# egordm/tch-geometric

Measured on AMD Instinct MI355X. Metric: sampled edges/sec, neighbor_sampling_homogenous fanout [15,10] on RMAT-24, higher is better.
Workload: dtype int64

## Files before the change

### tch-geometric_amd/csrc/ns_homo_win.hip

```cpp
#include <stdlib.h>

#include <algorithm>
#include <mutex>
#include <type_traits>

#include "ns_tickets.h"
#include "stage_bits.h"
#include "tg_device.h"
#include "tg_host.h"

namespace tg {

constexpr int WIN_PART_BLOCKS = 512;
constexpr int WIN_PART_THREADS = 512;
constexpr int WIN_TILE = 4096;
constexpr int WIN_MAX_BUCKETS = 8192;
constexpr int WIN_MAX_ROWS = 1024;
constexpr int WIN_MAX_PARTS = 16;

struct WinState {
    int64_t begin, end, ne, fbase;
};

struct WinQueues {
// ... 665 lines not shown
    return v ? atoi(v) : dflt;
}

struct WinTuning {
    int64_t window_bytes;
    int32_t gather_blocks, gather_threads, emit_threads, direct_hop0, fuse_first_hops, fold_hist, emit_blocks;
    int32_t staged, stage_round_chunks, stage_gather_threads, stage_gather_blocks, stage_emit_threads, stage_parts, stage_part_min_batches, stage_sort_blocks;
    int32_t stage_fine, stage_concurrent, stage_split, stage_split_round_chunks, store_align64, stage_fine_sub_bits, stage_fine_blocks;
};
static WinTuning &win_tuning() {
    static WinTuning t = {
        (int64_t)win_env_int("TG_WIN_KIB", 512) * 1024,
        win_env_int("TG_WIN_GATHER_BLOCKS", 256),
        win_env_int("TG_WIN_GATHER_THREADS", 512),
        win_env_int("TG_WIN_EMIT_THREADS", 256),
        win_env_int("TG_WIN_DIRECT_HOP0", 1),
        win_env_int("TG_WIN_FUSE_FIRST_HOPS", 1),
        win_env_int("TG_WIN_FOLD_HIST", 1),
        win_env_int("TG_WIN_EMIT_BLOCKS", 768),
        win_env_int("TG_WIN_STAGED", 2),
        win_env_int("TG_WIN_STAGE_ROUND_CHUNKS", 2),
        win_env_int("TG_WIN_STAGE_GATHER_THREADS", 512),
        win_env_int("TG_WIN_STAGE_GATHER_BLOCKS", 512),
        win_env_int("TG_WIN_STAGE_EMIT_THREADS", 256),
        win_env_int("TG_WIN_STAGE_PARTS", 1),
        win_env_int("TG_WIN_STAGE_PART_MIN_BATCHES", 1024),
        win_env_int("TG_WIN_STAGE_SORT_BLOCKS", 0),
        win_env_int("TG_WIN_STAGE_FINE", 1),
        win_env_int("TG_WIN_STAGE_CONCURRENT", 0),
        win_env_int("TG_WIN_STAGE_SPLIT", 0),
        win_env_int("TG_WIN_STAGE_SPLIT_ROUND_CHUNKS", 4),
        win_env_int("TG_WIN_STORE_ALIGN64", 1),
        win_env_int("TG_WIN_STAGE_FINE_SUB_BITS", 7),
        win_env_int("TG_WIN_STAGE_FINE_BLOCKS", 2048),
    };
    return t;
}

constexpr int WIN_MAX_STAGES = 8 * TG_MAX_HOPS + 2;
struct WinStageClock {
    bool enabled = false;
    int n = 0;
    hipEvent_t ev[WIN_MAX_STAGES + 1] = {};
    char name[WIN_MAX_STAGES][24] = {};
    void begin(hipStream_t s) {
        n = 0;
        if (!enabled) return;
        if (!ev[0])
            for (auto &e : ev) (void)hipEventCreate(&e);
        (void)hipEventRecord(ev[0], s);
    }
    void mark(const char *what, int hop, hipStream_t s) {
        if (!enabled || n >= WIN_MAX_STAGES) return;
        snprintf(name[n], sizeof(name[n]), "%s.h%d", what, hop);
        ++n;
        (void)hipEventRecord(ev[n], s);
    }
};
static WinStageClock &win_clock() {
    static WinStageClock c;
    return c;
}

struct WinLayout {
    size_t state, call_keys, n_items, queues, hist, base, items_in, items_sorted, vtab, fine_tot, fine_start, fine_tile_off, item_keys, stage, total, total_push;
    int64_t max_items;
    int stage_words;
};

static StageBits win_stage_bits(const tg_graph *csc) {
    StageBits sb;
    if (!csc) {
        sb.bv = sb.bp = 32;
        return sb;
    }
    sb.bv = stage_bits_of((uint64_t)std::max<int64_t>(csc->n_major, 1) - 1);
    const int64_t longest = csc->max_degree > 0 ? csc->max_degree : csc->n_edges;
    sb.bp = stage_bits_of((uint64_t)std::max<int64_t>(longest, 1) - 1);
    return sb;
}
static int win_stage_words(const tg_graph *csc, const int64_t *fanout, int32_t n_hops) {
    int64_t k = 0;
    for (int h = 1; h < n_hops; ++h) k = std::max(k, fanout[h]);
    if (n_hops < 2 || k > 32) return 0;
    if (!csc) return 32;
    const int bits = stage_slot_bits((int)k, win_stage_bits(csc));
    return (bits <= 512 && k <= 16) ? 16 : (bits <= 1024 ? 32 : 0);
}

static WinLayout win_layout(const tg_graph *csc, int64_t n_batches, int64_t n_seeds, const int64_t *fanout, int32_t n_hops) {
    WinLayout L;
    int64_t layer = n_seeds, widest = n_seeds;
    for (int h = 0; h + 1 < n_hops; ++h) {
        layer *= fanout[h];
        if (layer > widest) widest = layer;
    }
    L.max_items = n_batches * widest;
    size_t at = 0;
    auto take = [&](size_t bytes) {
        const size_t here = at;
        at += (bytes + 255) & ~(size_t)255;
        return here;
    };
    L.state = take((size_t)n_batches * sizeof(WinState));
    L.call_keys = take((size_t)n_batches * sizeof(CallKey));
    L.n_items = take(TG_MAX_HOPS * sizeof(unsigned long long));
    L.queues = take(WIN_MAX_PARTS * sizeof(WinQueues));
    L.hist = take((size_t)std::max(WIN_MAX_ROWS, WIN_MAX_PARTS * WIN_PART_BLOCKS) * WIN_MAX_BUCKETS * sizeof(uint32_t));
    L.base = take((size_t)WIN_MAX_PARTS * (WIN_MAX_BUCKETS + 8) * sizeof(uint32_t));
    L.items_in = take((size_t)L.max_items * sizeof(WinItemW));
    L.items_sorted = take((size_t)L.max_items * sizeof(WinItemW));
    L.vtab = take((size_t)(WIN_MAX_BUCKETS + 8) * sizeof(uint32_t));
    L.total_push = at;
    L.fine_tot = take((size_t)WIN_MAX_PARTS * (WIN_MAX_BUCKETS / 8 + 8) * WIN_FINE_PER_COARSE_MAX * sizeof(uint32_t));
    L.fine_start = take((size_t)WIN_MAX_PARTS * (WIN_MAX_BUCKETS / 8 + 8) * WIN_FINE_PER_COARSE_MAX * sizeof(uint32_t));
    L.fine_tile_off = take(((size_t)L.max_items / WIN_FINE_TILE + WIN_MAX_PARTS + 1) * WIN_FINE_BINS_MAX * sizeof(uint32_t));
    L.item_keys = take((size_t)L.max_items * sizeof(uint16_t));
    L.stage_words = win_stage_words(csc, fanout, n_hops);
    L.stage = take((size_t)L.max_items * L.stage_words * sizeof(uint32_t));
    L.total = at;
    return L;
}

template <typename Item, int KMAX, bool REPLACE>
static int win_run(WinParams p, int64_t n_batches, const int64_t *fanout, int32_t n_hops, hipStream_t stream) {
    const WinTuning t = win_tuning();
    WinStageClock &clk = win_clock();
    const int gather_blocks = (t.gather_blocks + 7) & ~7;
    const bool fold = t.fold_hist && t.direct_hop0 && t.fuse_first_hops && n_hops > 1;
    const size_t hist_lds = fold ? (size_t)p.n_buckets * sizeof(uint32_t) : 0;
    auto emit_threads_for = [&]() {
        int threads = t.emit_threads;
        while (threads > 64 && win_emit_lds_bytes(p.kmax, threads / 64) + hist_lds > 64 * 1024)
            threads = ((threads >> 1) + 63) & ~63;
        return threads;
    };
    p.n_batches = n_batches;
    p.n_rows = (int32_t)std::min<int64_t>(std::min(std::max(t.emit_blocks, 1), WIN_MAX_ROWS), n_batches);
    auto pitch_of = [&](int h) {
        int64_t f = p.n_seeds;
        for (int j = 0; j < h; ++j) f *= fanout[j];
        return f;
    };
    clk.begin(stream);
    int h0 = 0;
    if (t.direct_hop0 && t.fuse_first_hops) {
        const int threads = emit_threads_for();
        if (fold) {
            p.item_pitch = pitch_of(1);
            hipLaunchKernelGGL((win_first_hops_fold_kernel<Item, KMAX, REPLACE>), dim3((unsigned)p.n_rows), dim3(threads),
                               win_emit_lds_bytes(p.kmax, threads / 64) + hist_lds, stream, p, (int)fanout[0], (int)fanout[1]);
        } else {
            TG_HIP(hipMemsetAsync(p.n_items, 0, TG_MAX_HOPS * sizeof(unsigned long long), stream));
            hipLaunchKernelGGL((win_first_hops_kernel<Item, KMAX, REPLACE>), dim3((unsigned)n_batches), dim3(threads),
                               win_emit_lds_bytes(p.kmax, threads / 64), stream, p, (int)fanout[0],
                               n_hops > 1 ? (int)fanout[1] : 0);
        }
        TG_LAUNCH_CHECK();
        clk.mark("first_hops", 0, stream);
        h0 = 1;
    } else {
        hipLaunchKernelGGL(win_init_kernel, dim3((unsigned)n_batches), dim3(256), 0, stream, p, n_batches);
        TG_LAUNCH_CHECK();
        clk.mark("init", 0, stream);
    }
    for (int h = h0; h < n_hops; ++h) {
        p.hop = h;
        p.k = (int32_t)fanout[h];
        p.item_pitch = pitch_of(h);
        const bool emitted = (h == 1 && h0 == 1);
        if (!emitted) {
            const int threads = emit_threads_for();
            if (h == 0 && t.direct_hop0) {
                hipLaunchKernelGGL((win_emit_kernel<Item, KMAX, REPLACE, true>), dim3((unsigned)n_batches), dim3(threads),
                                   win_emit_lds_bytes(p.kmax, threads / 64), stream, p);
                TG_LAUNCH_CHECK();
                clk.mark("emit_direct", h, stream);
                continue;
            }
            if (fold)
                hipLaunchKernelGGL((win_emit_fold_kernel<Item, KMAX, REPLACE>), dim3((unsigned)p.n_rows), dim3(threads),
                                   win_emit_lds_bytes(p.kmax, threads / 64) + hist_lds, stream, p);
            else
                hipLaunchKernelGGL((win_emit_kernel<Item, KMAX, REPLACE, false>), dim3((unsigned)n_batches),
                                   dim3(threads), win_emit_lds_bytes(p.kmax, threads / 64), stream, p);
            TG_LAUNCH_CHECK();
            clk.mark("emit", h, stream);
        }
        if (!fold) {
            hipLaunchKernelGGL(win_hist_kernel<Item>, dim3(WIN_PART_BLOCKS), dim3(WIN_PART_THREADS), 0, stream, p);
            TG_LAUNCH_CHECK();
            clk.mark("hist", h, stream);
        }
        hipLaunchKernelGGL(win_colscan_kernel, dim3((p.n_buckets + 63) / 64), dim3(64 * WIN_SCAN_GROUPS), 0, stream, p,
                           fold ? p.n_rows : WIN_PART_BLOCKS);
        TG_LAUNCH_CHECK();
        hipLaunchKernelGGL(win_basescan_kernel, dim3(1), dim3(1024), 0, stream, p);
        TG_LAUNCH_CHECK();
        clk.mark("scans", h, stream);
        if (fold)
            hipLaunchKernelGGL(win_scatter_fold_kernel<Item>, dim3((unsigned)p.n_rows), dim3(WIN_PART_THREADS), 0, stream, p);
        else
            hipLaunchKernelGGL(win_scatter_kernel<Item>, dim3(WIN_PART_BLOCKS), dim3(WIN_PART_THREADS), 0, stream, p);
        TG_LAUNCH_CHECK();
        clk.mark("scatter", h, stream);
        int gthreads = t.gather_threads;
        while (gthreads > 64 && (size_t)(gthreads / 64) * win_gather_wave_lds_bytes(p.kmax) > 64 * 1024)
            gthreads = ((gthreads >> 1) + 63) & ~63;
        hipLaunchKernelGGL((win_gather_kernel<Item, KMAX, REPLACE>), dim3(gather_blocks), dim3(gthreads),
                           (size_t)(gthreads / 64) * win_gather_wave_lds_bytes(p.kmax), stream, p);
        TG_LAUNCH_CHECK();
        clk.mark("gather", h, stream);
    }
    return TG_OK;
}

constexpr int64_t WIN_STAGED_AUTO_MIN_BATCHES = 2048;
static bool win_staged_wanted(const WinTuning &t, int64_t n_batches, int stage_words) {
    if (t.staged == 2) return n_batches >= WIN_STAGED_AUTO_MIN_BATCHES && stage_words == 16;
    return t.staged != 0;
}
static bool win_staged_applicable(const WinParams &p, const WinTuning &t, const tg_graph *csc, int64_t n_batches,
                                  const int64_t *fanout, int32_t n_hops, int stage_words) {
    if (!win_staged_wanted(t, n_batches, stage_words) || !t.direct_hop0 || n_hops < 2 || stage_words == 0) return false;
    if (csc->n_major >= ((int64_t)1 << 32) || csc->n_edges >= ((int64_t)1 << 32)) return false;
    int64_t pitch = p.n_seeds;
    for (int h = 1; h < n_hops; ++h) {
        pitch *= fanout[h - 1];
        int bits = 1;
        while (((int64_t)1 << bits) < pitch) ++bits;
        if (bits >= 32 || n_batches > ((int64_t)1 << (32 - bits))) return false;
    }
    return true;
}

struct WinSide {
    hipStream_t stream = nullptr;
    hipEvent_t gathered[WIN_MAX_PARTS] = {}, done = nullptr;
    std::mutex mu;
    int ensure() {
        if (stream) return TG_OK;
        int least = 0, greatest = 0;
        const int prio = win_env_int("TG_WIN_SIDE_PRIO", 1);
        if (prio && hipDeviceGetStreamPriorityRange(&least, &greatest) == hipSuccess && greatest < least)
            TG_HIP(hipStreamCreateWithPriority(&stream, hipStreamNonBlocking, prio == 2 ? least : greatest));
        else
            TG_HIP(hipStreamCreateWithFlags(&stream, hipStreamNonBlocking));
        for (auto &e : gathered) TG_HIP(hipEventCreateWithFlags(&e, hipEventDisableTiming));
        TG_HIP(hipEventCreateWithFlags(&done, hipEventDisableTiming));
        return TG_OK;
    }
};
static WinSide &win_side() {
    static WinSide s;
    return s;
}

struct WinDeviceLds {
    int cus, per_cu, per_block;
};
static int win_device_lds(WinDeviceLds *out) {
    constexpr int MAX_DEV = 64;
    static std::mutex mu;
    static WinDeviceLds known[MAX_DEV];
    static bool have[MAX_DEV] = {};
    int dev = 0;
    TG_HIP(hipGetDevice(&dev));
    std::lock_guard<std::mutex> lock(mu);
    if (dev < 0 || dev >= MAX_DEV || !have[dev]) {
        WinDeviceLds d;
        TG_HIP(hipDeviceGetAttribute(&d.cus, hipDeviceAttributeMultiprocessorCount, dev));
        TG_HIP(hipDeviceGetAttribute(&d.per_cu, hipDeviceAttributeMaxSharedMemoryPerMultiprocessor, dev));
        TG_HIP(hipDeviceGetAttribute(&d.per_block, hipDeviceAttributeMaxSharedMemoryPerBlock, dev));
        if (dev < 0 || dev >= MAX_DEV) {
            *out = d;
            return TG_OK;
        }
        known[dev] = d;
        have[dev] = true;
    }
    *out = known[dev];
    return TG_OK;
}

static size_t win_stage_first_lds(int kmax, int threads, int n_coarse, int n_windows, bool narrow) {
    return win_emit_lds_bytes(kmax, threads / 64, WIN_STAGE_FIRST_RC, narrow) + win_stage_tables_bytes(n_coarse, n_windows);
}
static int win_stage_first_threads(int emit_threads, int kmax, int n_coarse, int n_windows, bool narrow) {
    int threads = std::min(emit_threads, WIN_EMIT_MAX_THREADS);
    while (threads > 64 && win_stage_first_lds(kmax, threads, n_coarse, n_windows, narrow) > 64 * 1024)
        threads = ((threads >> 1) + 63) & ~63;
    return threads;
}

struct WinFirstLaunch {
    int32_t rows = 0, per_cu = 0, threads = 0, narrow = 0;
    int64_t lds_bytes = 0;
};
static WinFirstLaunch &win_first_launch() {
    static WinFirstLaunch f;
    return f;
}

template <int W, int KFIRST, int KMAX, bool REPLACE>
static int win_run_staged(WinParams p, const tg_graph *csc, int64_t n_batches, const int64_t *fanout, int32_t n_hops,
                          hipStream_t stream) {
    const WinTuning t = win_tuning();
    WinStageClock &clk = win_clock();
    const StageBits sb = win_stage_bits(csc);
    p.n_windows = (int32_t)((csc->n_edges >> p.shift) + 1);
    auto pitch_of = [&](int h) {
        int64_t f = p.n_seeds;
        for (int j = 0; j < h; ++j) f *= fanout[j];
        return f;
    };
    auto bits_of = [&](int64_t pitch) {
        int bits = 1;
        while (((int64_t)1 << bits) < pitch) ++bits;
        return bits;
    };
    p.n_wbuckets = (p.n_buckets + 63) & ~63;
    p.n_buckets = p.n_wbuckets >> 3;
    const size_t tables = win_stage_tables_bytes(p.n_buckets, p.n_windows);
    int parts = std::min(std::max(t.stage_parts, 1), WIN_MAX_PARTS);
    while (parts > 1 && n_batches / parts < std::max(t.stage_part_min_batches, 1)) --parts;
    if (clk.enabled) parts = 1;
    const bool split = t.stage_split && !clk.enabled;
    if (split) parts = 1;
    WinSide &side = win_side();
    std::unique_lock<std::mutex> side_lock(side.mu, std::defer_lock);
    if (parts > 1 || split) {
        side_lock.lock();
        const int rc = side.ensure();
        if (rc != TG_OK) return rc;
    }
    uint32_t *const hist0 = p.hist, *const base0 = p.base;
    WinQueues *const queues0 = p.queues;
    void *const sorted0 = p.items_sorted, *const in0 = p.items_in;
    uint32_t *const fine_tot0 = p.fine_tot, *const fine_start0 = p.fine_start, *const fine_tile_off0 = p.fine_tile_off;
    const bool first_in_parts = parts > 1 && n_hops == 2;

    WinDeviceLds dl;
    {
        const int rc = win_device_lds(&dl);
        if (rc != TG_OK) return rc;
    }
    const bool narrow_cols = p.ptrs32 != nullptr;
    const int fthreads = win_stage_first_threads(t.emit_threads, p.kmax, p.n_buckets, p.n_windows, narrow_cols);
    const size_t flds = win_stage_first_lds(p.kmax, fthreads, p.n_buckets, p.n_windows, narrow_cols);
    int first_per_cu = 0;
    if (t.stage_sort_blocks <= 0) {
        struct Seen {
            int dev = -1, threads = 0, narrow = 0, per_cu = 0;
            size_t lds = 0;
        };
        static Seen seen;
        static std::mutex seen_mu;
        int dev = 0;
        TG_HIP(hipGetDevice(&dev));
        std::lock_guard<std::mutex> lock(seen_mu);
        if (seen.dev != dev || seen.threads != fthreads || seen.narrow != (int)narrow_cols || seen.lds != flds) {
            const int by_lds = (int)((size_t)dl.per_cu / flds), by_regs = (4 * (512 / 128)) / (fthreads / 64);
            int by_runtime = 0;
            if (narrow_cols)
                TG_HIP(hipOccupancyMaxActiveBlocksPerMultiprocessor(&by_runtime, win_stage_first_kernel<KFIRST, REPLACE, true>, fthreads, flds));
            else
                TG_HIP(hipOccupancyMaxActiveBlocksPerMultiprocessor(&by_runtime, win_stage_first_kernel<KFIRST, REPLACE, false>, fthreads, flds));
            seen.dev = dev;
            seen.threads = fthreads;
            seen.narrow = (int)narrow_cols;
            seen.lds = flds;
            seen.per_cu = std::max(1, std::min(std::min(by_lds, by_regs), by_runtime > 0 ? by_runtime : 1));
        }
        first_per_cu = seen.per_cu;
    }
    const int64_t rows_wanted = t.stage_sort_blocks > 0 ? (int64_t)t.stage_sort_blocks : (int64_t)first_per_cu * std::max(dl.cus, 1);
    auto rows_of = [&](int64_t nb) {
        return (int32_t)std::min<int64_t>(std::min<int64_t>(std::max<int64_t>(rows_wanted, 1), WIN_MAX_ROWS), nb);
    };
    auto part_tables = [&](int part) {
        p.hist = hist0 + (size_t)part * WIN_MAX_ROWS * (WIN_MAX_BUCKETS / 8);
        p.base = base0 + (size_t)part * (WIN_MAX_BUCKETS + 8);
        p.queues = queues0 + part;
    };
    auto launch_first = [&](int part, int64_t b0, int64_t nb, hipStream_t ps) {
        part_tables(part);
        p.b0 = b0;
        p.n_batches = nb;
        p.n_rows = rows_of(nb);
        p.next_pitch = pitch_of(1);
        p.next_idx_bits = bits_of(p.next_pitch);
        if (narrow_cols)
            hipLaunchKernelGGL((win_stage_first_kernel<KFIRST, REPLACE, true>), dim3((unsigned)p.n_rows), dim3(fthreads), flds, ps,
                               p, (int)fanout[0]);
        else
            hipLaunchKernelGGL((win_stage_first_kernel<KFIRST, REPLACE, false>), dim3((unsigned)p.n_rows), dim3(fthreads), flds, ps,
                               p, (int)fanout[0]);
        WinFirstLaunch &fl = win_first_launch();
        fl.rows = p.n_rows;
        fl.per_cu = first_per_cu;
        fl.threads = fthreads;
        fl.narrow = (int32_t)narrow_cols;
        fl.lds_bytes = (int64_t)flds;
    };
    const bool concurrent = first_in_parts && t.stage_concurrent;

    clk.begin(stream);
    hipLaunchKernelGGL(win_vtab_kernel, dim3((p.n_windows + 256) / 256), dim3(256), 0, stream, p, csc->n_major);
    TG_LAUNCH_CHECK();
    if (!first_in_parts) {
        launch_first(0, 0, n_batches, stream);
        TG_LAUNCH_CHECK();
        clk.mark("first", 0, stream);
    }
    if (concurrent) {
        TG_HIP(hipEventRecord(side.gathered[0], stream));
        TG_HIP(hipStreamWaitEvent(side.stream, side.gathered[0], 0));
    }
    for (int h = 1; h < n_hops; ++h) {
        const bool next = h + 1 < n_hops;
        const int hparts = next ? 1 : parts;
        for (int part = 0; part < hparts; ++part) {
            const int64_t b0 = n_batches * part / hparts, nb = n_batches * (part + 1) / hparts - b0;
            const bool counted = h == 1 && (first_in_parts || hparts == 1);
            hipStream_t ps = (concurrent && (part & 1)) ? side.stream : stream;
            if (first_in_parts) {
                launch_first(part, b0, nb, ps);
                TG_LAUNCH_CHECK();
            }
            p.hop = h;
            p.k = (int32_t)fanout[h];
            p.item_pitch = pitch_of(h);
            p.idx_bits = bits_of(p.item_pitch);
            p.next_pitch = next ? pitch_of(h + 1) : 0;
            p.next_idx_bits = next ? bits_of(p.next_pitch) : 0;
            int ethreads = t.stage_emit_threads;
            int rc = std::min(std::max(split ? t.stage_split_round_chunks : t.stage_round_chunks, 1), WIN_STAGE_ROUND_CHUNKS_MAX);
            while (win_stage_emit_lds_bytes(W, p.k, ethreads / 64, rc, split) > 64 * 1024) {
                if (rc > 1)
                    rc >>= 1;
                else if (ethreads > 64)
                    ethreads = ((ethreads >> 1) + 63) & ~63;
                else
                    return tg::fail(TG_ERR_INVALID, "tg_ns_homo_batched_ws: the staged emit kernel does not fit the LDS");
            }
            const size_t elds = win_stage_emit_lds_bytes(W, p.k, ethreads / 64, rc, split);
            int gthreads = t.stage_gather_threads;
            const size_t per_wave = (size_t)(64 * (W + 1) + 64) * sizeof(uint32_t);
            const size_t gcap = std::max<size_t>(64 * 1024, std::min<size_t>((size_t)std::max(dl.per_block, 0), 128 * 1024));
            while (gthreads > 64 && (size_t)(gthreads / 64) * per_wave > gcap) gthreads = ((gthreads >> 1) + 63) & ~63;
            if ((size_t)(gthreads / 64) * per_wave > 64 * 1024) {
                static int raised_on = -1;
                int dev = 0;
                TG_HIP(hipGetDevice(&dev));
                if (raised_on != dev) {
                    TG_HIP(hipFuncSetAttribute(reinterpret_cast<const void *>(&win_stage_gather_kernel<W, KMAX, REPLACE>),
                                               hipFuncAttributeMaxDynamicSharedMemorySize, (int)gcap));
                    raised_on = dev;
                }
            }
            const int gblocks = (std::max(t.stage_gather_blocks, 8) + 7) & ~7;
            part_tables(part);
            p.b0 = b0;
            p.n_batches = nb;
            p.n_rows = rows_of(nb);
            p.items_in = in0;
            p.items_sorted = static_cast<WinItem8 *>(sorted0) + p.b0 * p.item_pitch;
            p.items_fine = static_cast<WinItem8 *>(in0) + p.b0 * p.item_pitch;
            if (!counted) {
                hipLaunchKernelGGL(win_hist8_kernel, dim3((unsigned)p.n_rows), dim3(WIN_PART_THREADS), tables, ps, p);
                TG_LAUNCH_CHECK();
                clk.mark("hist", h, stream);
            }
            hipLaunchKernelGGL(win_colscan_kernel, dim3((p.n_buckets + 63) / 64), dim3(64 * WIN_SCAN_GROUPS), 0, ps, p,
                               p.n_rows);
            TG_LAUNCH_CHECK();
            hipLaunchKernelGGL(win_basescan_kernel, dim3(1), dim3(1024), 0, ps, p);
            TG_LAUNCH_CHECK();
            clk.mark("scans", h, stream);
            {
                static const int tiled = win_env_int("TG_WIN_SCATTER_TILED", 1);
                static const int carry = win_env_int("TG_WIN_SCATTER_CARRY", 1);
                const size_t clds = win_scatter8_carry_lds(WIN_SC_CARRY_TILE, p.n_buckets);
                const size_t ccap = std::max<size_t>(64 * 1024, std::min<size_t>((size_t)std::max(dl.per_block, 0), 128 * 1024));
                if (tiled && carry && p.n_buckets <= WIN_PART_THREADS && clds <= ccap) {
                    if (clds > 64 * 1024) {
                        static int raised_on = -1;
                        int dev = 0;
                        TG_HIP(hipGetDevice(&dev));
                        if (raised_on != dev) {
                            TG_HIP(hipFuncSetAttribute(reinterpret_cast<const void *>(&win_scatter8_carry_kernel<WIN_SC_CARRY_TILE>),
                                                       hipFuncAttributeMaxDynamicSharedMemorySize, (int)ccap));
                            raised_on = dev;
                        }
                    }
                    hipLaunchKernelGGL(win_scatter8_carry_kernel<WIN_SC_CARRY_TILE>, dim3((unsigned)p.n_rows), dim3(WIN_PART_THREADS), clds,
                                       ps, p);
                } else if (tiled && p.n_buckets <= WIN_PART_THREADS && win_scatter8_tiled_lds(p.n_buckets, p.n_windows) <= 64 * 1024)
                    hipLaunchKernelGGL(win_scatter8_tiled_kernel, dim3((unsigned)p.n_rows), dim3(WIN_PART_THREADS),
                                       win_scatter8_tiled_lds(p.n_buckets, p.n_windows), ps, p);
                else
                    hipLaunchKernelGGL(win_scatter8_kernel, dim3((unsigned)p.n_rows), dim3(WIN_PART_THREADS), tables, ps, p);
            }
            TG_LAUNCH_CHECK();
            clk.mark("scatter", h, stream);
            if (t.stage_fine) {
                const int64_t worst = p.n_batches * p.item_pitch;
                const size_t vt = (size_t)(p.n_windows + 1 + p.n_buckets + 1) * sizeof(uint32_t);
                p.fine_sub_bits = std::min(std::max(t.stage_fine_sub_bits, 4), WIN_FINE_SUB_BITS_MAX);
                const int per_coarse = 8 << p.fine_sub_bits;
                const size_t keys = (size_t)(p.n_buckets + 1) * per_coarse;
                p.fine_tot = fine_tot0 + (size_t)part * (WIN_MAX_BUCKETS / 8 + 8) * WIN_FINE_PER_COARSE_MAX;
                p.fine_start = fine_start0 + (size_t)part * (WIN_MAX_BUCKETS / 8 + 8) * WIN_FINE_PER_COARSE_MAX;
                p.fine_tile_off = fine_tile_off0 + ((size_t)(p.b0 * p.item_pitch) / WIN_FINE_TILE + (size_t)part) * WIN_FINE_BINS_MAX;
                p.fine_rowtot = p.fine_start + (size_t)(WIN_MAX_BUCKETS / 8 + 1) * WIN_FINE_PER_COARSE_MAX;
                const unsigned tiles = (unsigned)std::max<int64_t>(1, std::min<int64_t>((worst + WIN_FINE_TILE - 1) / WIN_FINE_TILE, t.stage_fine_blocks));
                TG_HIP(hipMemsetAsync(p.fine_tot, 0, keys * sizeof(uint32_t), ps));
                hipLaunchKernelGGL(win_sort_fine_kernel<false>, dim3(tiles), dim3(WIN_FINE_THREADS), vt, ps, p);
                TG_LAUNCH_CHECK();
                hipLaunchKernelGGL(win_fine_rowsum_kernel, dim3((p.n_buckets + 16) / 16), dim3(1024), 0, ps, p);
                TG_LAUNCH_CHECK();
                hipLaunchKernelGGL(win_fine_starts_kernel, dim3((p.n_buckets + 16) / 16), dim3(1024), 0, ps, p);
                TG_LAUNCH_CHECK();
                hipLaunchKernelGGL(win_sort_fine_kernel<true>, dim3(tiles), dim3(WIN_FINE_THREADS), vt, ps, p);
                TG_LAUNCH_CHECK();
                clk.mark("fine", h, stream);
            } else
                p.items_fine = p.items_sorted;
            if (split) TG_HIP(hipEventRecord(side.gathered[h & (WIN_MAX_PARTS - 1)], ps));
            hipLaunchKernelGGL((win_stage_gather_kernel<W, KMAX, REPLACE>), dim3(gblocks), dim3(gthreads),
                               (size_t)(gthreads / 64) * per_wave, ps, p, sb);
            TG_LAUNCH_CHECK();
            if (split) {
                int sthreads = std::min(t.emit_threads, WIN_EMIT_MAX_THREADS);
                while (sthreads > 64 && win_emit_lds_bytes(p.kmax, sthreads / 64, WIN_STAGE_SIDE_RC) > 64 * 1024) sthreads = ((sthreads >> 1) + 63) & ~63;
                TG_HIP(hipStreamWaitEvent(side.stream, side.gathered[h & (WIN_MAX_PARTS - 1)], 0));
                hipLaunchKernelGGL((win_stage_side_kernel<KMAX, REPLACE>), dim3((unsigned)p.n_batches), dim3(sthreads),
                                   win_emit_lds_bytes(p.kmax, sthreads / 64, WIN_STAGE_SIDE_RC), side.stream, p);
                TG_LAUNCH_CHECK();
                TG_HIP(hipEventRecord(side.done, side.stream));
            }
            clk.mark("gather", h, stream);
            hipStream_t es = ps;
            if (split) TG_HIP(hipStreamWaitEvent(ps, side.done, 0));
            if (hparts > 1 && !concurrent) {
                TG_HIP(hipEventRecord(side.gathered[part], stream));
                TG_HIP(hipStreamWaitEvent(side.stream, side.gathered[part], 0));
                es = side.stream;
            }
            if (split) {
                if (next)
                    hipLaunchKernelGGL((win_stage_emit_kernel<W, KMAX, true, true>), dim3((unsigned)p.n_batches),
                                       dim3(ethreads), elds, es, p, sb, rc);
                else
                    hipLaunchKernelGGL((win_stage_emit_kernel<W, KMAX, false, true>), dim3((unsigned)p.n_batches),
                                       dim3(ethreads), elds, es, p, sb, rc);
            } else if (next)
                hipLaunchKernelGGL((win_stage_emit_kernel<W, KMAX, true, false>), dim3((unsigned)p.n_batches), dim3(ethreads),
                                   elds, es, p, sb, rc);
            else
                hipLaunchKernelGGL((win_stage_emit_kernel<W, KMAX, false, false>), dim3((unsigned)p.n_batches), dim3(ethreads),
                                   elds, es, p, sb, rc);
            TG_LAUNCH_CHECK();
            clk.mark("emit", h, stream);
        }
        if (hparts > 1) {
            TG_HIP(hipEventRecord(side.done, side.stream));
            TG_HIP(hipStreamWaitEvent(stream, side.done, 0));
        }
    }
    return TG_OK;
}

template <bool REPLACE>
static int win_dispatch_staged(const WinParams &p, const tg_graph *csc, int stage_words, int64_t n_batches,
                               const int64_t *fanout, int32_t n_hops, hipStream_t stream) {
    int64_t kord = 0;
    for (int h = 1; h < n_hops; ++h) kord = std::max(kord, fanout[h]);
    if (stage_words == 16 && kord <= 12)
        return fanout[0] <= 16 ? win_run_staged<16, 16, 12, REPLACE>(p, csc, n_batches, fanout, n_hops, stream)
                               : win_run_staged<16, 32, 12, REPLACE>(p, csc, n_batches, fanout, n_hops, stream);
    if (stage_words == 16)
        return fanout[0] <= 16 ? win_run_staged<16, 16, 16, REPLACE>(p, csc, n_batches, fanout, n_hops, stream)
                               : win_run_staged<16, 32, 16, REPLACE>(p, csc, n_batches, fanout, n_hops, stream);
    return fanout[0] <= 16 ? win_run_staged<32, 16, 32, REPLACE>(p, csc, n_batches, fanout, n_hops, stream)
                           : win_run_staged<32, 32, 32, REPLACE>(p, csc, n_batches, fanout, n_hops, stream);
}

static void win_window_geometry(const tg_graph *csc, int32_t *shift_out, int32_t *n_buckets_out) {
    const int elem = csc->indices32 ? 4 : 8;
    int shift = 0;
    while (((int64_t)elem << shift) < win_tuning().window_bytes) ++shift;
    while (((csc->n_edges >> shift) + 1) > WIN_MAX_BUCKETS - 8) ++shift;
    int32_t nb = (int32_t)((((csc->n_edges >> shift) + 1) + 7) & ~(int64_t)7);
    if (nb < 8) nb = 8;
    *shift_out = shift;
    *n_buckets_out = nb;
}

template <typename Item>
static int win_dispatch(const WinParams &p, bool repl, int64_t n_batches, const int64_t *fanout, int32_t n_hops,
                        hipStream_t stream) {
    if (p.kmax <= 16)
        return repl ? win_run<Item, 16, true>(p, n_batches, fanout, n_hops, stream)
                    : win_run<Item, 16, false>(p, n_batches, fanout, n_hops, stream);
    return repl ? win_run<Item, 32, true>(p, n_batches, fanout, n_hops, stream)
                : win_run<Item, 32, false>(p, n_batches, fanout, n_hops, stream);
}

}

extern "C" int tg_ns_homo_workspace_bytes_for(const tg_graph *csc, int64_t n_batches, int64_t n_seeds, const int64_t *fanout,
                                              int32_t n_hops, int64_t *n_bytes) {
    TG_REQUIRE(n_batches >= 0 && n_seeds >= 0 && n_hops >= 0 && n_hops <= TG_MAX_HOPS && (fanout || n_hops == 0) &&
                   n_bytes,
               "tg_ns_homo_workspace_bytes: bad arguments");
    for (int h = 0; h < n_hops; ++h)
        TG_REQUIRE(fanout[h] >= 1 && fanout[h] <= 255, "tg_ns_homo_workspace_bytes: fanout[%d] outside [1, 255]", h);
    const tg::WinLayout L = tg::win_layout(csc, n_batches, n_seeds, fanout, n_hops);
    const tg::WinTuning &t = tg::win_tuning();
    const bool staged = csc ? tg::win_staged_wanted(t, n_batches, L.stage_words)
                            : (t.staged == 2 ? n_batches >= tg::WIN_STAGED_AUTO_MIN_BATCHES && L.stage_words != 0
                                             : t.staged != 0);
    *n_bytes = (int64_t)(staged ? L.total : L.total_push);
    return TG_OK;
}
extern "C" int tg_ns_homo_workspace_bytes(int64_t n_batches, int64_t n_seeds, const int64_t *fanout, int32_t n_hops,
                                          int64_t *n_bytes) {
    return tg_ns_homo_workspace_bytes_for(nullptr, n_batches, n_seeds, fanout, n_hops, n_bytes);
}

int tg_ns_homo_windowed_applicable(const tg_graph *csc, int64_t n_batches, int64_t n_seeds, const int64_t *fanout,
                                   int32_t n_hops, const tg_ns_config *cfg, const tg_ns_out *out, int32_t mode) {
    if (mode == TG_NS_FORM_FUSED) return 0;
    const int sampler = cfg ? cfg->sampler : TG_SAMPLER_UNIFORM;
    const int filter = cfg ? cfg->filter_mode : TG_FILTER_NONE;
    if (sampler == TG_SAMPLER_WEIGHTED || filter != TG_FILTER_NONE) return 0;
    if (sampler == TG_SAMPLER_LABOR || sampler == TG_SAMPLER_LABOR_SHARED) return 0;
    if (cfg && (cfg->seed_ids || cfg->seed_call_ids)) return 0;
    if (n_hops < 1 || n_batches < 1 || n_seeds < 1) return 0;
    int kmax = 1;
    for (int h = 0; h < n_hops; ++h) kmax = fanout[h] > kmax ? (int)fanout[h] : kmax;
    if (kmax > TG_MAX_FANOUT) return 0;
    const tg::WinLayout L = tg::win_layout(csc, n_batches, n_seeds, fanout, n_hops);
    if (L.max_items >= ((int64_t)1 << 32) || out->cap_nodes >= ((int64_t)1 << 32) || n_batches >= ((int64_t)1 << 32))
        return 0;
    if (mode == TG_NS_FORM_WINDOWED || mode == TG_NS_FORM_WINDOWED_WIDE) return 1;
    return n_batches * n_seeds >= ((int64_t)1 << 21) && csc->n_edges >= ((int64_t)1 << 24);
}

int tg_ns_homo_windowed_launch(const tg_graph *csc, const int64_t *seeds, int64_t n_batches, int64_t n_seeds,
                               const int64_t *fanout, int32_t n_hops, const tg_ns_config *cfg, const tg_rng *rng,
                               const tg_ns_out *out, void *ws, int64_t ws_bytes, int32_t mode, hipStream_t stream) {
    using namespace tg;
    const WinLayout L = win_layout(csc, n_batches, n_seeds, fanout, n_hops);
    TG_REQUIRE(ws && ws_bytes >= (int64_t)L.total_push, "tg_ns_homo_batched_ws: workspace too small (%lld < %lld bytes)",
               (long long)ws_bytes, (long long)L.total_push);
    TG_REQUIRE(((uintptr_t)ws & 255) == 0, "tg_ns_homo_batched_ws: workspace must be 256-byte aligned");
    TG_REQUIRE((((uintptr_t)out->samples | (uintptr_t)out->rows | (uintptr_t)out->cols | (uintptr_t)out->edge_index) & 7u) == 0,
               "tg_ns_homo_batched_ws: output slabs must be 8-byte aligned");
    WinParams p;
    p.store_align = win_tuning().store_align64 ? 7u : 1u;

    p.ptrs = csc->ptrs;
    p.indices = csc->indices;
    p.indices32 = csc->indices32;
    p.ptrs32 = csc->ptrs32;
    p.seeds = seeds;
    p.n_seeds = n_seeds;
    p.n_hops = n_hops;
    p.hop = 0;
    p.k = 0;
    p.kmax = 1;
    for (int h = 0; h < n_hops; ++h) p.kmax = fanout[h] > p.kmax ? (int32_t)fanout[h] : p.kmax;
    p.cap_nodes = out->cap_nodes;
    p.cap_edges = out->cap_edges;
    p.samples = out->samples;
    p.rows = ns_rows_prefilled(out, n_seeds) ? nullptr : out->rows;
    p.cols = out->cols;
    p.edge_index = out->edge_index;
    p.layer_offsets = out->layer_offsets;
    p.counts = out->counts;
    p.seed = rng->seed;
    p.call_id = rng->call_id;
    p.tag = (cfg && cfg->rng_tag) ? cfg->rng_tag : TG_TAG_NS_HOMO;
    p.id_base = cfg ? cfg->id_base : 0;
    TG_BOUNDS_INIT(p, csc);
    unsigned char *w = static_cast<unsigned char *>(ws);
    p.state = reinterpret_cast<WinState *>(w + L.state);
    p.call_keys = reinterpret_cast<CallKey *>(w + L.call_keys);
    p.n_items = reinterpret_cast<unsigned long long *>(w + L.n_items);
    p.queues = reinterpret_cast<WinQueues *>(w + L.queues);
    p.hist = reinterpret_cast<uint32_t *>(w + L.hist);
    p.base = reinterpret_cast<uint32_t *>(w + L.base);
    p.items_in = w + L.items_in;
    p.items_sorted = w + L.items_sorted;
    win_window_geometry(csc, &p.shift, &p.n_buckets);
    int slot_bits = 1;
    while (((int64_t)1 << slot_bits) < out->cap_nodes) ++slot_bits;
    const bool narrow = csc->n_edges < ((int64_t)1 << 32) && out->cap_edges < ((int64_t)1 << 32) && slot_bits < 32 &&
                        n_batches <= ((int64_t)1 << (32 - slot_bits));
    const bool force_wide = mode == TG_NS_FORM_WINDOWED_WIDE;
    p.slot_bits = slot_bits;
    const bool repl = (cfg ? cfg->sampler : TG_SAMPLER_UNIFORM) == TG_SAMPLER_UNIFORM_REPL;
    p.vtab = reinterpret_cast<uint32_t *>(w + L.vtab);
    p.fine_tot = reinterpret_cast<uint32_t *>(w + L.fine_tot);
    p.fine_start = reinterpret_cast<uint32_t *>(w + L.fine_start);
    p.fine_tile_off = reinterpret_cast<uint32_t *>(w + L.fine_tile_off);
    p.item_keys = reinterpret_cast<uint16_t *>(w + L.item_keys);
    p.stage = reinterpret_cast<uint32_t *>(w + L.stage);
    if (narrow && !force_wide && ws_bytes >= (int64_t)L.total &&
        win_staged_applicable(p, win_tuning(), csc, n_batches, fanout, n_hops, L.stage_words))
        return repl ? win_dispatch_staged<true>(p, csc, L.stage_words, n_batches, fanout, n_hops, stream)
                    : win_dispatch_staged<false>(p, csc, L.stage_words, n_batches, fanout, n_hops, stream);
    if (narrow && !force_wide) return win_dispatch<WinItemN>(p, repl, n_batches, fanout, n_hops, stream);
    return win_dispatch<WinItemW>(p, repl, n_batches, fanout, n_hops, stream);
}

extern "C" int tg_ns_win_tuning_get(tg_ns_win_tuning *t) {
    TG_REQUIRE(t, "tg_ns_win_tuning_get: null");
    const tg::WinTuning &w = tg::win_tuning();
    t->window_bytes = w.window_bytes;
    t->gather_blocks = w.gather_blocks;
    t->gather_threads = w.gather_threads;
    t->emit_threads = w.emit_threads;
    t->direct_hop0 = w.direct_hop0;
    t->fuse_first_hops = w.fuse_first_hops;
    t->fold_hist = w.fold_hist;
    t->emit_blocks = w.emit_blocks;
    t->staged = w.staged;
    t->stage_round_chunks = w.stage_round_chunks;
    t->stage_gather_threads = w.stage_gather_threads;
    t->stage_gather_blocks = w.stage_gather_blocks;
    t->stage_emit_threads = w.stage_emit_threads;
    t->stage_parts = w.stage_parts;
    t->stage_part_min_batches = w.stage_part_min_batches;
    t->stage_sort_blocks = w.stage_sort_blocks > 0 ? w.stage_sort_blocks : -1;
    t->stage_fine = w.stage_fine;
    t->stage_concurrent = w.stage_concurrent;
    t->stage_split = w.stage_split;
    t->stage_split_round_chunks = w.stage_split_round_chunks;
    t->store_align64 = w.store_align64;
    t->stage_fine_sub_bits = w.stage_fine_sub_bits;
    t->stage_fine_blocks = w.stage_fine_blocks;
    return TG_OK;
}

extern "C" int tg_ns_win_tuning_set(const tg_ns_win_tuning *t) {
    TG_REQUIRE(t, "tg_ns_win_tuning_set: null");
    TG_REQUIRE(t->window_bytes == 0 || (t->window_bytes >= 64 && t->window_bytes <= ((int64_t)1 << 32)),
               "tg_ns_win_tuning_set: window_bytes outside [64, 2^32]");
    TG_REQUIRE(t->gather_threads == 0 || (t->gather_threads >= 64 && t->gather_threads <= 1024 && t->gather_threads % 64 == 0),
               "tg_ns_win_tuning_set: gather_threads must be a multiple of 64 in [64, 1024]");
    TG_REQUIRE(t->emit_threads == 0 || (t->emit_threads >= 64 && t->emit_threads <= 1024 && t->emit_threads % 64 == 0),
               "tg_ns_win_tuning_set: emit_threads must be a multiple of 64 in [64, 1024]");
    TG_REQUIRE(t->gather_blocks >= 0 && t->gather_blocks <= 65536, "tg_ns_win_tuning_set: gather_blocks outside [0, 65536]");
    tg::WinTuning &w = tg::win_tuning();
    if (t->window_bytes) w.window_bytes = t->window_bytes;
    if (t->gather_blocks) w.gather_blocks = t->gather_blocks;
    if (t->gather_threads) w.gather_threads = t->gather_threads;
    if (t->emit_threads) w.emit_threads = t->emit_threads;
    if (t->direct_hop0 >= 0) w.direct_hop0 = t->direct_hop0 != 0;
    if (t->fuse_first_hops >= 0) w.fuse_first_hops = t->fuse_first_hops != 0;
    if (t->fold_hist >= 0) w.fold_hist = t->fold_hist != 0;
    if (t->emit_blocks > 0) w.emit_blocks = t->emit_blocks;
    if (t->staged >= 0) w.staged = t->staged > 2 ? 1 : t->staged;
    if (t->stage_round_chunks > 0) w.stage_round_chunks = t->stage_round_chunks;
    if (t->stage_gather_threads >= 64 && t->stage_gather_threads <= 1024) w.stage_gather_threads = t->stage_gather_threads & ~63;
    if (t->stage_gather_blocks > 0) w.stage_gather_blocks = t->stage_gather_blocks;
    if (t->stage_emit_threads >= 64 && t->stage_emit_threads <= 1024) w.stage_emit_threads = t->stage_emit_threads & ~63;
    if (t->stage_parts > 0) w.stage_parts = t->stage_parts;
    if (t->stage_part_min_batches > 0) w.stage_part_min_batches = t->stage_part_min_batches;
    if (t->stage_sort_blocks != 0) w.stage_sort_blocks = t->stage_sort_blocks > 0 ? t->stage_sort_blocks : 0;
    if (t->stage_fine >= 0) w.stage_fine = t->stage_fine != 0;
    if (t->stage_concurrent >= 0) w.stage_concurrent = t->stage_concurrent != 0;
    if (t->stage_split >= 0) w.stage_split = t->stage_split != 0;
    if (t->stage_split_round_chunks > 0) w.stage_split_round_chunks = t->stage_split_round_chunks;
    if (t->store_align64 >= 0) w.store_align64 = t->store_align64 != 0;
    if (t->stage_fine_sub_bits > 0) w.stage_fine_sub_bits = std::min(std::max(t->stage_fine_sub_bits, 4), tg::WIN_FINE_SUB_BITS_MAX);
    if (t->stage_fine_blocks > 0) w.stage_fine_blocks = std::min((t->stage_fine_blocks + 7) & ~7, 8192);
    return TG_OK;
}

extern "C" int tg_ns_win_first_lds_bytes(int32_t emit_threads, int32_t kmax, int32_t n_coarse_buckets, int32_t n_windows,
                                         int32_t narrow, int32_t *threads, int64_t *lds_bytes) {
    TG_REQUIRE(lds_bytes && emit_threads >= 64 && emit_threads <= 1024 && emit_threads % 64 == 0 && kmax >= 1 && kmax <= TG_MAX_FANOUT &&
                   n_coarse_buckets >= 0 && n_windows >= 0,
               "tg_ns_win_first_lds_bytes: bad arguments");
    const int th = tg::win_stage_first_threads(emit_threads, kmax, n_coarse_buckets, n_windows, narrow != 0);
    if (threads) *threads = th;
    *lds_bytes = (int64_t)tg::win_stage_first_lds(kmax, th, n_coarse_buckets, n_windows, narrow != 0);
    return TG_OK;
}

extern "C" int tg_ns_win_first_launch(int32_t *rows, int32_t *workgroups_per_cu, int32_t *threads, int32_t *narrow, int64_t *lds_bytes) {
    const tg::WinFirstLaunch &f = tg::win_first_launch();
    if (rows) *rows = f.rows;
    if (workgroups_per_cu) *workgroups_per_cu = f.per_cu;
    if (threads) *threads = f.threads;
    if (narrow) *narrow = f.narrow;
    if (lds_bytes) *lds_bytes = f.lds_bytes;
    return TG_OK;
}

extern "C" int tg_ns_win_stage_timing(int32_t enable) {
    tg::win_clock().enabled = enable != 0;
    return TG_OK;
}

extern "C" int tg_ns_win_stage_times(float *ms, char *names, int32_t cap, int32_t *n) {
    TG_REQUIRE(n && (cap == 0 || (ms && names)), "tg_ns_win_stage_times: null arguments");
    tg::WinStageClock &c = tg::win_clock();
    *n = c.n;
    if (c.n == 0) return TG_OK;
    TG_HIP(hipEventSynchronize(c.ev[c.n]));
    for (int i = 0; i < c.n && i < cap; ++i) {
        TG_HIP(hipEventElapsedTime(&ms[i], c.ev[i], c.ev[i + 1]));
        snprintf(names + (size_t)i * 24, 24, "%s", c.name[i]);
    }
    return TG_OK;
}

extern "C" int tg_ns_homo_batched_form(const tg_graph *csc, int64_t n_batches, int64_t n_seeds, const int64_t *fanout,
                                       int32_t n_hops, const tg_ns_config *cfg, const tg_ns_out *out,
                                       int64_t workspace_bytes, int32_t mode, int32_t *form, int32_t *n_windows) {
    TG_REQUIRE(csc && out && form && (fanout || n_hops == 0), "tg_ns_homo_batched_form: null arguments");
    TG_REQUIRE(n_hops >= 0 && n_hops <= TG_MAX_HOPS, "tg_ns_homo_batched_form: n_hops %d outside [0, %d]", n_hops, TG_MAX_HOPS);
    *form = TG_NS_FORM_FUSED;
    if (n_windows) *n_windows = 0;
    const int sampler = cfg ? cfg->sampler : TG_SAMPLER_UNIFORM;
    const int filter = cfg ? cfg->filter_mode : TG_FILTER_NONE;
    if (sampler == TG_SAMPLER_WEIGHTED || filter != TG_FILTER_NONE) return TG_OK;
    if (sampler == TG_SAMPLER_LABOR || sampler == TG_SAMPLER_LABOR_SHARED) return TG_OK;
    if (workspace_bytes <= 0 || !tg_ns_homo_windowed_applicable(csc, n_batches, n_seeds, fanout, n_hops, cfg, out, mode))
        return TG_OK;
    if ((int64_t)tg::win_layout(csc, n_batches, n_seeds, fanout, n_hops).total_push > workspace_bytes) return TG_OK;
    int32_t shift = 0, nb = 0;
    tg::win_window_geometry(csc, &shift, &nb);
    int slot_bits = 1;
    while (((int64_t)1 << slot_bits) < out->cap_nodes) ++slot_bits;
    const bool narrow = csc->n_edges < ((int64_t)1 << 32) && out->cap_edges < ((int64_t)1 << 32) && slot_bits < 32 &&
                        n_batches <= ((int64_t)1 << (32 - slot_bits));
    *form = (narrow && mode != TG_NS_FORM_WINDOWED_WIDE) ? TG_NS_FORM_WINDOWED : TG_NS_FORM_WINDOWED_WIDE;
    if (n_windows) *n_windows = nb;
    return TG_OK;
}

extern "C" int tg_ns_homo_batched_pipeline(const tg_graph *csc, int64_t n_batches, int64_t n_seeds, const int64_t *fanout,
                                           int32_t n_hops, const tg_ns_config *cfg, const tg_ns_out *out,
                                           int64_t workspace_bytes, int32_t mode, int32_t *staged) {
    TG_REQUIRE(staged, "tg_ns_homo_batched_pipeline: null");
    *staged = 0;
    int32_t form = 0, n_win = 0;
    const int rc = tg_ns_homo_batched_form(csc, n_batches, n_seeds, fanout, n_hops, cfg, out, workspace_bytes, mode, &form, &n_win);
    if (rc != TG_OK || form != TG_NS_FORM_WINDOWED) return rc;
    const tg::WinLayout L = tg::win_layout(csc, n_batches, n_seeds, fanout, n_hops);
    tg::WinParams p{};
    p.n_seeds = n_seeds;
    *staged = workspace_bytes >= (int64_t)L.total &&
              tg::win_staged_applicable(p, tg::win_tuning(), csc, n_batches, fanout, n_hops, L.stage_words);
    return TG_OK;
}
```

Measured before the change: 81.74 billion.

## Add list and run variants of fine sort kernel with larger LDS

Selects among new template variants of the fine-sort kernel (per-bin lists and run-based placement) through env flags that default to on. When the placement pass's LDS need exceeds 64 KiB, it raises the kernel's dynamic shared memory limit to up to 128 KiB. The goal is cheaper fine-bucket sorting and placement by keeping more state in LDS. The larger LDS footprint may reduce occupancy. The kernel template changes live elsewhere, so this shows only the host side. It also stops rounding the fine block count to a multiple of 8.

```diff
diff --git a/tch-geometric_amd/csrc/ns_homo_win.hip b/tch-geometric_amd/csrc/ns_homo_win.hip
--- a/tch-geometric_amd/csrc/ns_homo_win.hip
+++ b/tch-geometric_amd/csrc/ns_homo_win.hip
@@ -991,6 +991,13 @@
     return f;
 }
 
+using WinFineKernel = void (*)(const WinParams);
+static WinFineKernel win_sort_fine_pick(bool place, bool lists, bool runs) {
+    if (!place) return lists ? win_sort_fine_kernel<false, true, false> : win_sort_fine_kernel<false, false, false>;
+    if (runs) return lists ? win_sort_fine_kernel<true, true, true> : win_sort_fine_kernel<true, false, true>;
+    return lists ? win_sort_fine_kernel<true, true, false> : win_sort_fine_kernel<true, false, false>;
+}
+
 template <int W, int KFIRST, int KMAX, bool REPLACE>
 static int win_run_staged(WinParams p, const tg_graph *csc, int64_t n_batches, const int64_t *fanout, int32_t n_hops,
                           hipStream_t stream) {
@@ -1195,7 +1202,6 @@
             clk.mark("scatter", h, stream);
             if (t.stage_fine) {
                 const int64_t worst = p.n_batches * p.item_pitch;
-                const size_t vt = (size_t)(p.n_windows + 1 + p.n_buckets + 1) * sizeof(uint32_t);
                 p.fine_sub_bits = std::min(std::max(t.stage_fine_sub_bits, 4), WIN_FINE_SUB_BITS_MAX);
                 const int per_coarse = 8 << p.fine_sub_bits;
                 const size_t keys = (size_t)(p.n_buckets + 1) * per_coarse;
@@ -1204,14 +1210,33 @@
                 p.fine_tile_off = fine_tile_off0 + ((size_t)(p.b0 * p.item_pitch) / WIN_FINE_TILE + (size_t)part) * WIN_FINE_BINS_MAX;
                 p.fine_rowtot = p.fine_start + (size_t)(WIN_MAX_BUCKETS / 8 + 1) * WIN_FINE_PER_COARSE_MAX;
                 const unsigned tiles = (unsigned)std::max<int64_t>(1, std::min<int64_t>((worst + WIN_FINE_TILE - 1) / WIN_FINE_TILE, t.stage_fine_blocks));
+                const bool f_lists = win_env_int("TG_WIN_FINE_LISTS", 1) != 0;
+                const size_t fcap = std::max<size_t>(64 * 1024, std::min<size_t>((size_t)std::max(dl.per_block, 0), 128 * 1024));
+                const bool f_runs = win_env_int("TG_WIN_FINE_RUNS", 1) != 0 && win_sort_fine_lds(p.n_windows, p.n_buckets, true) <= fcap;
+                auto fine_pass = [&](bool place) -> int {
+                    const bool runs = place && f_runs;
+                    const WinFineKernel kern = win_sort_fine_pick(place, f_lists, runs);
+                    const size_t lds = win_sort_fine_lds(p.n_windows, p.n_buckets, runs);
+                    if (lds > 64 * 1024) {
+                        static int raised_on[2] = {-1, -1};
+                        int dev = 0;
+                        TG_HIP(hipGetDevice(&dev));
+                        if (raised_on[f_lists] != dev) {
+                            TG_HIP(hipFuncSetAttribute(reinterpret_cast<const void *>(kern), hipFuncAttributeMaxDynamicSharedMemorySize, (int)fcap));
+                            raised_on[f_lists] = dev;
+                        }
+                    }
+                    hipLaunchKernelGGL(kern, dim3(tiles), dim3(WIN_FINE_THREADS), lds, ps, p);
+                    return TG_OK;
+                };
                 TG_HIP(hipMemsetAsync(p.fine_tot, 0, keys * sizeof(uint32_t), ps));
-                hipLaunchKernelGGL(win_sort_fine_kernel<false>, dim3(tiles), dim3(WIN_FINE_THREADS), vt, ps, p);
+                if (const int rc = fine_pass(false); rc != TG_OK) return rc;
                 TG_LAUNCH_CHECK();
                 hipLaunchKernelGGL(win_fine_rowsum_kernel, dim3((p.n_buckets + 16) / 16), dim3(1024), 0, ps, p);
                 TG_LAUNCH_CHECK();
                 hipLaunchKernelGGL(win_fine_starts_kernel, dim3((p.n_buckets + 16) / 16), dim3(1024), 0, ps, p);
                 TG_LAUNCH_CHECK();
-                hipLaunchKernelGGL(win_sort_fine_kernel<true>, dim3(tiles), dim3(WIN_FINE_THREADS), vt, ps, p);
+                if (const int rc = fine_pass(true); rc != TG_OK) return rc;
                 TG_LAUNCH_CHECK();
                 clk.mark("fine", h, stream);
             } else
@@ -1467,7 +1492,7 @@
     if (t->stage_split_round_chunks > 0) w.stage_split_round_chunks = t->stage_split_round_chunks;
     if (t->store_align64 >= 0) w.store_align64 = t->store_align64 != 0;
     if (t->stage_fine_sub_bits > 0) w.stage_fine_sub_bits = std::min(std::max(t->stage_fine_sub_bits, 4), tg::WIN_FINE_SUB_BITS_MAX);
-    if (t->stage_fine_blocks > 0) w.stage_fine_blocks = std::min((t->stage_fine_blocks + 7) & ~7, 8192);
+    if (t->stage_fine_blocks > 0) w.stage_fine_blocks = std::min(t->stage_fine_blocks, 8192);
     return TG_OK;
 }
 
```

Measured after the change: 82.41 billion (median of 6 runs). Within noise of the previous version (+0.8%).
